# var-nan/SGUFP_Solver

Measured on AMD Instinct MI355X. Metric: B&B-node relaxations/sec + achieved HBM GB/s, 1k-arc 256-scenario synthetic, higher is better.
Workload: dtype f64; 1 GPU; C4: 1000-arc layered network, 256 scenarios, 16F+64O pool, BFS frontier of 8192 open nodes per GPU; instance_seed=1, nodes_per_gpu=8192, total_layers=281, parallelism=frontier shards x1

## Files before the change

include/sgufp_hip.h:

```cpp
#ifndef SGUFP_HIP_H
#define SGUFP_HIP_H

#include <stdint.h>

#ifdef __cplusplus
extern "C" {
#endif

typedef struct sgufp_ctx sgufp_ctx;

#define SGUFP_OK 0
#define SGUFP_ERR_ARG (-1)
#define SGUFP_ERR_NETWORK (-2)
#define SGUFP_ERR_HIP (-3)
#define SGUFP_ERR_CAPACITY (-4)
#define SGUFP_ERR_STATE (-5)
#define SGUFP_ERR_KEY (-6)

#define SGUFP_SUCCESS 0
#define SGUFP_PRUNED_BY_FEASIBILITY_CUT 1
#define SGUFP_PRUNED_BY_OPTIMALITY_CUT 2
#define SGUFP_NEEDS_SUBPROBLEM 3
#define SGUFP_PRUNED_BY_BOUND 4
#define SGUFP_NODE_ERR_RECORD 16
// ... 41 lines not shown
int sgufp_batch_children(sgufp_ctx *ctx, int64_t *child_off, uint16_t *global_layer, double *lb, double *ub,
                         int64_t *states_off, int16_t *states, int64_t *sol_off, int16_t *sol);
int sgufp_batch_paths(sgufp_ctx *ctx, int64_t *path_off, int16_t *paths);
int sgufp_batch_stats(sgufp_ctx *ctx, int64_t *dd_nodes, int64_t *dd_arcs, int32_t *dd_layers, int32_t *sweeps);
int sgufp_batch_refine(sgufp_ctx *ctx, int n, const int32_t *node_idx, const uint8_t *is_feasibility,
                       const int32_t *cut_index, double optimal_lb);

int sgufp_dd_build(sgufp_ctx *ctx);
int sgufp_dd_apply(sgufp_ctx *ctx, int node, int is_feasibility, double rhs, int64_t nnz, const uint64_t *keys,
                   const double *vals, double optimal, double *value);
int sgufp_dd_solution(sgufp_ctx *ctx, int node, int16_t *path, int32_t *len);
int sgufp_dd_cutset(sgufp_ctx *ctx, int node, double ub, int64_t *n_children);

int sgufp_batch_debug(sgufp_ctx *ctx, int64_t *ticks, int32_t *redo);
int sgufp_relax_launches(const sgufp_ctx *ctx, int64_t *launches);
int sgufp_batch_phases(sgufp_ctx *ctx, int64_t *phase);
int sgufp_batch_narrow_split(sgufp_ctx *ctx, int64_t *split);
int sgufp_batch_refold_stats(sgufp_ctx *ctx, uint32_t *stats);

#define SGUFP_ROUTE_IN_ORDER 0
#define SGUFP_ROUTE_EXACT_PHASE 1
#define SGUFP_ROUTE_NX_PHASE 2
#define SGUFP_ROUTE_NX_FALLBACK 3
int sgufp_batch_routes(sgufp_ctx *ctx, int32_t *route);

int sgufp_subproblem(sgufp_ctx *ctx, int n, const int64_t *path_off, const int16_t *paths, int32_t *type,
                     double *rhs, double *rows, double *obj_mean);
int sgufp_subproblem_detail(sgufp_ctx *ctx, int32_t *status, double *objective, double *dual_objective);
int sgufp_subproblem_warm(sgufp_ctx *ctx, int n, const int64_t *path_off, const int16_t *paths, const int32_t *warm_src,
                          const int32_t *warm_dst, int32_t *type, double *rhs, double *rows, double *obj_mean);
// ... 87 lines not shown
```

sgufp_solver_amd/csrc/capi.cpp:

```cpp
#include <cstdio>

#include "ctx.hpp"
#include <algorithm>
#include <cstdlib>


namespace {

int64_t node_bound(const Network &net, int64_t *tail = nullptr) {
    const int L = net.L;
    auto set_size = [&](int sid) { return sid >= 0 ? (int)net.sets[sid].size() : 1; };
    int start = std::max(0, L - 5);
    std::vector<int64_t> h(kMaxStates + 2, 0);
    int c0 = set_size(net.layer_universe[start]);
    h[c0] = (L > 5) ? kRelaxedMaxWidth - 1 : 1;
    int64_t total = (int64_t)(kRelaxedMaxWidth - 1) * (start + 1);
    int64_t tail_nodes = 0;
    for (int l = start; l < L; l++) {
        if (net.layer_update[l] >= 0) {
            int64_t w = 0;
            for (auto x : h) w += x;
            std::fill(h.begin(), h.end(), 0);
            h[set_size(net.layer_update[l])] = w;
        }
// ... 88 lines not shown
    if (const char *e = getenv("SGUFP_NX_MIN")) nx_min = std::max(1, atoi(e));
    if (const char *e = getenv("SGUFP_NX_SKIP")) nx_skip = std::max(0, atoi(e));
    if (const char *e = getenv("SGUFP_REDO_SWEEP")) sc.redo_sweep = atoi(e) != 0;
    if (const char *e = getenv("SGUFP_RELAX_CHUNK")) { split_q = std::max(0, atoi(e)); split_forced = true; }
    if (const char *e = getenv("SGUFP_RELAX_STREAMS")) split_parts = std::max(1, std::min(kRelaxMaxParts, atoi(e)));
    int64_t acap = std::max<int64_t>(1, (int64_t)std::max(0, L - 4) * (kRelaxedMaxWidth - 1) * maxU);
    if (ncap > (int64_t)kParentMask || acap > (int64_t)0x7FFFFFFF) { err = "DD capacity beyond 22-bit indices"; return false; }
    sc.Ncap = (int)ncap;
    sc.Acap = (int)acap;
    sc.us = ustride;
    if (net.n_slots >= 32767) { err = "more than 32766 coefficient slots (int16 root-solution slots)"; return false; }
    if (relax_lds_bytes(sc.Tcap, sc.Lcap, cb, sc.us) > 160 * 1024) { err = "too many layers for the LDS layer table"; return false; }
    sc.tmir_cap = cb > 1 ? (int)(sc.Ncap + sc.Acap) : 0;
    sc.tail_cap = (int)tail;
    sc.cb_max = cb;
    const size_t B = (size_t)max_batch;
    if (!alloc(sc.ntopo, B * sc.Ncap, "scratch") || !alloc(sc.nflag, B * sc.Ncap, "scratch") ||
        !alloc(sc.nmask, B * sc.Ncap, "scratch") || !alloc(sc.outcnt, B * sc.Ncap, "scratch") ||
        !alloc(sc.s2, B * sc.Ncap, "scratch") || !alloc(sc.tw, B * sc.Ncap, "scratch") ||
        !alloc(sc.atopo, B * sc.Acap, "scratch") || !alloc(sc.aflag, B * sc.Acap, "scratch") ||
        !alloc(sc.lay, B * sc.Tcap * 5, "scratch") || !alloc(sc.rslot, B * sc.Lcap, "scratch") ||
        !alloc(sc.meta, B * 8, "scratch") || !alloc(sc.ubv, B, "scratch") ||
        !alloc(sc.sm1, B * sc.Tcap, "scratch") || !alloc(sc.xm1, B * sc.Tcap, "scratch") ||
        !alloc(sc.v1, B * sc.Tcap, "scratch"))
        return false;
    if (cb > 1 && (!alloc(sc.s2b, B * sc.tail_cap * cb, "scratch") || !alloc(sc.sm, B * sc.Tcap * cb, "scratch") ||
                   !alloc(sc.xm, B * sc.Tcap * cb, "scratch") || !alloc(sc.tmir, B * (size_t)sc.tmir_cap, "scratch")))
        return false;
    if (cb > 1 && split_q > 0) {
        if (!alloc(sc.resume, B * kResumeWords, "scratch") || !alloc(sc.rgs, B * (size_t)(sc.Tcap + 1), "scratch")) return false;
        split_min = cus * relax_occupancy(sc.Tcap, sc.Lcap, cb, sc.us) * 3 / 2;
    }
    if (const char *e = getenv("SGUFP_REFOLD_STATS"))
        if (atoi(e) != 0 && cb > 1 && !alloc(sc.rstat, B * kRefoldStats, "scratch")) return false;
    if (!alloc(out.status, B, "out") || !alloc(out.exact, B, "out") || !alloc(out.lb, B, "out") ||
        !alloc(out.ub, B, "out") || !alloc(out.nchild, B, "out") || !alloc(out.sol_need, B, "out") ||
        !alloc(out.dd_nodes, B, "out") || !alloc(out.dd_arcs, B, "out") || !alloc(out.dd_layers, B, "out") ||
        !alloc(out.sweeps, B, "out") || !alloc(out.path, B * sc.Lcap, "out") || !alloc(out.path_len, B, "out") ||
        !alloc(out.ticks, B, "out") || !alloc(out.redo, B, "out") || !alloc(out.phase, B * kPhaseSlots, "out"))
        return false;
    if (!alloc(d_gl, B, "batch") || !alloc(d_sollen, B, "batch") || !alloc(d_lb, B, "batch") ||
        !alloc(d_ub, B, "batch") || !alloc(d_mask, B, "batch") || !alloc(d_valid, B, "batch") ||
        !alloc(d_soloff, B, "batch") || !alloc(d_coff, B + 1, "batch") || !alloc(d_soff, B + 1, "batch") ||
        !alloc(d_rslots, B, "batch") || !alloc(d_rcuts, B, "batch") || !alloc(d_rfeas, B, "batch"))
        return false;
    sol_cap = B * (size_t)std::max(1, L);
    if (!alloc(d_sol, sol_cap, "batch")) return false;
// ... 232 lines not shown
        if (!alloc(d_G, B * (size_t)ocap, "nx gaps") || !alloc(d_MS, B * (size_t)ocap, "nx maxState")) return false;
        nx_cap = ocap;
    }
    ex.nx = 1;
    ex.pkind = d_pkind;
    ex.P = d_P;
    ex.G = d_G;
    ex.MS = d_MS;
    ex.nxh = d_nxh;
    ex.pstop = d_pstop;
    ex.nxlist = d_nxlist;
    ex.nx_ms = 0;
    return true;
}

bool sgufp_ctx::split_prepare() {
    if (split_ready) return true;
    if (!hip_ok(hipEventCreateWithFlags(&split.fork, hipEventDisableTiming), "event")) return false;
    for (int k = 0; k + 1 < split_parts; k++)
        if (!hip_ok(hipStreamCreateWithFlags(&split.extra[k], hipStreamNonBlocking), "stream") ||
            !hip_ok(hipEventCreateWithFlags(&split.join[k], hipEventDisableTiming), "event"))
            return false;
    split_ready = true;
    return true;
}

bool sgufp_ctx::relax_current(double optimal_lb) {
    dd_built = false;
    if (!push_orders() || !exact_prepare()) return false;
    relax_lb = optimal_lb;
    BatchIn in = cur;
    if (!relax_order(in)) return false;
    const Pool p = pool();
    hipStream_t st = stream;
    const bool do_split = sc.resume && split_q > 0 && (split_forced || in.n >= split_min);
    if (do_split && !split_prepare()) return false;
    split.q = do_split ? split_q : 0;
    split.parts = split_parts;
    relax_launches = 0;
    split.launches = &relax_launches;
    if (timing) hipEventRecord(ev[0], st);
    if (!hip_ok(launch_relax(nd, sc, in, p, out, optimal_lb, cb, ex, cus, st, &split), "k_relax")) return false;
    if (timing) hipEventRecord(ev[1], st);
    return emit_current(in, p);
}

bool sgufp_ctx::emit_current(const BatchIn &in, const Pool &p) {
    hipStream_t st = stream;
    if (in.n > 0 && !hip_ok(launch_scan(out.nchild, out.sol_need, in.n, d_coff, d_soff, st), "k_scan2")) return false;
    uint64_t tot[2] = {0, 0};
    if (in.n > 0) {
        if (!download(&tot[0], d_coff + in.n, 1) || !download(&tot[1], d_soff + in.n, 1)) return false;
    }
    if (!sync()) return false;
    const char *es = std::getenv("SGUFP_EXACT_STATS");
    const bool estats = es && es[0] == '1';
    if (estats && ex.enabled) {
// ... 901 lines not shown
        const auto &v = is_feasibility[k] ? ctx->f_rows : ctx->o_rows;
        if (node_idx[k] < 0 || node_idx[k] >= ctx->n || cut_index[k] < 0 || cut_index[k] >= (int)v.size())
            return SGUFP_ERR_ARG;
        rows[k] = v[cut_index[k]];
    }
    if (!ctx->upload(ctx->d_rslots, node_idx, n) || !ctx->upload(ctx->d_rcuts, rows.data(), n) ||
        !ctx->upload(ctx->d_rfeas, is_feasibility, n))
        return SGUFP_ERR_HIP;
    if (!ctx->hip_ok(launch_refine(ctx->nd, ctx->sc, ctx->batch(), ctx->pool(), ctx->out, ctx->d_rslots, ctx->d_rcuts,
                                   ctx->d_rfeas, n, optimal_lb, ctx->ex, ctx->stream),
                     "k_refine"))
        return SGUFP_ERR_HIP;
    return ctx->sync() ? SGUFP_OK : SGUFP_ERR_HIP;
}

int sgufp_relax_launches(const sgufp_ctx *ctx, int64_t *launches) {
    if (!ctx || !launches) return SGUFP_ERR_ARG;
    if (!ctx->relaxed) return SGUFP_ERR_STATE;
    *launches = (int64_t)ctx->relax_launches;
    return SGUFP_OK;
}

int sgufp_batch_phases(sgufp_ctx *ctx, int64_t *phase) {
    if (!ctx || !ctx->relaxed || !phase) return ctx ? SGUFP_ERR_STATE : SGUFP_ERR_ARG;
    if (!relax_has_phases()) {
        std::fill(phase, phase + (size_t)ctx->n * 8, (int64_t)0);
        return SGUFP_OK;
    }
    std::vector<uint64_t> t((size_t)ctx->n * kPhaseSlots);
    if (!ctx->download(t.data(), ctx->out.phase, t.size()) || !ctx->sync()) return SGUFP_ERR_HIP;
// ... 206 lines not shown
```

sgufp_solver_amd/csrc/ctx.hpp:

```cpp
#pragma once

#include "sgufp_hip.h"

#include <hip/hip_runtime.h>

#include <algorithm>
#include <cstdlib>
#include <cstring>
#include <memory>
#include <string>
#include <unordered_map>
#include <vector>

#define SGUFP_HOST_ONLY 1
#include "dd_device.hpp"
#include "network.hpp"
#include "sub_device.hpp"
#include "rdd_device.hpp"
#include "select_device.hpp"

namespace sgufp {
struct Transport;
size_t relax_lds_bytes(int Tcap, int Lcap, int cb, int us);
size_t sub_lds_bytes(int n, int m, int nct_cap, int nz, int nw, int kbytes = 8, bool warm = false);
hipError_t launch_subproblem(const SubNet &N, const SubIO &io, hipStream_t st);
hipError_t launch_warm_pick(const SubIO &io, const WarmRing &wr, int ptr, hipStream_t st);
hipError_t launch_flow_summary(int P, int S, int m, const int32_t *reward, int16_t *x, const uint8_t *ok,
                               double *flow_reward, double *mean_flow, hipStream_t st);
hipError_t launch_relax(const NetDev &, const Scratch &, const BatchIn &, const Pool &, const BatchOut &, double, int,
                        const ExactIO &, int, hipStream_t, const RelaxSplit *);
int relax_occupancy(int Tcap, int Lcap, int cb, int us);
hipError_t launch_exact_cols(const double *rows, const double *rhs, const int32_t *o_order, int no, int first,
                             int stride, int n_slots, int ostride, double *coefO, int reverse, hipStream_t st);
hipError_t launch_scan(const uint32_t *, const uint32_t *, int, uint64_t *, uint64_t *, hipStream_t);
hipError_t launch_emit(const NetDev &, const Scratch &, const BatchIn &, const Pool &, const BatchOut &,
                       const ChildOut &, hipStream_t);
hipError_t launch_refine(const NetDev &, const Scratch &, const BatchIn &, const Pool &, const BatchOut &,
                         const int32_t *, const int32_t *, const uint8_t *, int, double, const ExactIO &, hipStream_t);
hipError_t launch_gather_paths(const BatchOut &, int Lcap, const int32_t *idx, const int64_t *off, int n,
                               int16_t *dst, hipStream_t);
hipError_t launch_push_children(const ChildOut &, const BatchOut &, const int32_t *parents, const int64_t *dst_child,
                                const int64_t *dst_sol, int n, const FrontierDev &, hipStream_t);
hipError_t launch_dd_build(const NetDev &, const Scratch &, const BatchIn &, const BatchOut &, int stride, hipStream_t);
hipError_t launch_dd_apply(const NetDev &, const Scratch &, const BatchIn &, const BatchOut &, int slot, const double *rows,
                           int stride, double rhs, int is_feas, double optimal, double *value, hipStream_t);
// ... 206 lines not shown
    unsigned long long leaf_cum[5] = {0, 0, 0, 0, 0};
    int32_t *d_open_cnt = nullptr, *d_open_list = nullptr;
    double *d_G = nullptr;
    unsigned long long *d_MS = nullptr;
    int nx_cap = 0;
    bool nx_prepare(int no);
    bool exact_prepare();

    int split_q = 32, split_parts = 2, split_min = 0;
    bool split_forced = false;
    RelaxSplit split{};
    bool split_ready = false;
    bool split_prepare();
    unsigned long long relax_launches = 0;

    bool timing = false;
    hipEvent_t ev[4] = {};
    float ms_relax = 0, ms_emit = 0;

    ~sgufp_ctx();
    void destroy_all() {
        if (device >= 0) (void)hipSetDevice(device);
        for (auto &b : allocs) (void)hipFree(b.p);
        for (auto &e : ev)
            if (e) (void)hipEventDestroy(e);
        if (split.fork) (void)hipEventDestroy(split.fork);
        for (auto &e : split.join)
            if (e) (void)hipEventDestroy(e);
        for (auto &s : split.extra)
            if (s) (void)hipStreamDestroy(s);
// ... 88 lines not shown
```

sgufp_solver_amd/csrc/dd_device.hpp:

```cpp
#pragma once

#include <cstdint>

#include <hip/hip_runtime_api.h>

#if defined(__HIP_DEVICE_COMPILE__) && !defined(SGUFP_HOST_ONLY)
#define SGUFP_GBL __attribute__((address_space(1)))
#else
#define SGUFP_GBL
#endif

namespace sgufp {

constexpr int kWave = 64;
constexpr int kMaxU = 32;
constexpr int kLdsWidth = 512;
constexpr int kBoundBlocks = 1024;

enum NodeStatus : int32_t {
    kSuccess = 0,
    kPrunedFeasibility = 1,
    kPrunedOptimality = 2,
    kNeedsSubproblem = 3,
    kPrunedBound = 4,
// ... 65 lines not shown

constexpr int kRelaxWhole = 0, kRelaxHead = 1, kRelaxChunk = 2;
constexpr int32_t kRelaxPending = 8;
struct RelaxPart {
    int first;
    int q;
};
constexpr int kRelaxMaxParts = 4;
struct RelaxSplit {
    int q, parts;
    hipStream_t extra[kRelaxMaxParts - 1];
    hipEvent_t fork, join[kRelaxMaxParts - 1];
    unsigned long long *launches;
};

struct BatchIn {
    int n;
    const uint16_t SGUFP_GBL *gl;
    const double SGUFP_GBL *lb;
    const double SGUFP_GBL *ub;
    const uint32_t SGUFP_GBL *mask;
    const uint8_t SGUFP_GBL *valid;
    const int64_t SGUFP_GBL *sol_off;
    const uint16_t SGUFP_GBL *sol_len;
    const int16_t SGUFP_GBL *sol;
    int bound_prune;
    const int32_t SGUFP_GBL *perm;
};

struct FrontierDev {
// ... 125 lines not shown
```

sgufp_solver_amd/csrc/dd_kernels.hip:

```cpp
#include <hip/hip_runtime.h>

#include <algorithm>
#include <climits>
#include <cstdint>
#include <type_traits>

#include "dd_device.hpp"
#include "wave.hpp"

namespace sgufp {

#define DMIN (-__DBL_MAX__)
#define DMAX (__DBL_MAX__)

constexpr uint32_t kCollapseWidth = 120;


struct VP {
    double v;
    int p;
};
__device__ __forceinline__ VP vp_pick(VP a, VP b) {
    const bool take_b = (a.p == INT_MIN) | ((b.p != INT_MIN) & ((b.v > a.v) | (!(a.v > b.v) & (b.p > a.p))));
    VP r;
// ... 1556 lines not shown
__device__ __forceinline__ void store_meta_layers(const DD &d, const Scratch &sc, int slot, int last_cut, int status,
                                         int cut_layer, double ub) {
    GBL int32_t *meta = sc.meta + (size_t)slot * 8;
    if (lane() == 0) {
        meta[0] = d.g; meta[1] = d.len; meta[2] = d.T; meta[3] = d.exact; meta[4] = d.aligned;
        meta[5] = last_cut; meta[6] = status; meta[7] = cut_layer;
        sc.ubv[slot] = ub;
    }
    GBL uint32_t *lay = sc.lay + (size_t)slot * sc.Tcap * 5;
    for (int k = lane(); k < d.T; k += kWave) {
        lay[k] = (d.noff[k]); lay[sc.Tcap + k] = (d.nn[k]); lay[2 * sc.Tcap + k] = (d.nalive[k]);
        lay[3 * sc.Tcap + k] = (d.aoff[k]); lay[4 * sc.Tcap + k] = (d.acnt[k]);
    }
}

__device__ __forceinline__ int dd_solution_path(const NetDev &net, DD &d, const GBL double *row, GBL int16_t *out_path,
                                const GBL int16_t *rsol) {
    const int last = d.T - 1;
    const uint32_t lo = uni(d.noff[last]), ln = uni(d.nn[last]);
    VP best{0.0, INT_MIN};
    for (uint32_t base = 0; base < ln; base += kWave) {
        uint32_t i = base + lane();
        if (i < ln && (d.nflag[lo + i] & kAlive)) best = vp_pick(best, VP{d.tw[lo + i], prio_old((int)i)});
    }
    best = wave_vp(best);
    uint32_t node = 0;
    int k = 0;
    if (best.p != INT_MIN && best.v > DMIN) {
        node = lo + (uint32_t)(-best.p - 2);
        k = last;
// ... 597 lines not shown
    bv.tring = (LDS uint16_t *)(smem + cv.o_tring);
    bv.coef = (LDS double *)(smem + cv.o_bcoef);
    bv.w1 = smem + cv.o_w1;
    bv.ids = (LDS int32_t *)(smem + cv.o_ids);
    bv.wm = (LDS uint64_t *)(smem + cv.o_wm);
    bv.fm = bv.wm + (sc.Tcap + 63) / 64;
    bv.wsel = nullptr;
    bv.s2b = sc.s2b + (size_t)slot * sc.tail_cap * CB;
    bv.sm = sc.sm + (size_t)slot * sc.Tcap * CB;
    bv.xm = sc.xm + (size_t)slot * sc.Tcap * CB;
    bv.rstat = sc.rstat ? sc.rstat + (size_t)slot * kRefoldStats : nullptr;
}

template <int CB, int MODE = kRelaxWhole>
__global__ void __launch_bounds__(kWave, 2) k_relax(NetDev net, Scratch sc, BatchIn in, Pool pool, BatchOut out,
                                                double incumbent, ExactIO ex, RelaxPart part) {
    static_assert(MODE == kRelaxWhole || CB > 1, "only the batched loop suspends");
    extern __shared__ __attribute__((aligned(16))) uint8_t smem_raw[];
    LDS uint8_t *smem = (LDS uint8_t *)smem_raw;
    constexpr bool chunk = MODE == kRelaxChunk;
    const int wg = part.first + (int)blockIdx.x;
    if (wg >= in.n) return;
    const int slot = in.perm ? in.perm[wg] : wg;
    if (MODE == kRelaxWhole && ex.redo && out.status[slot] != kNxFallback) return;
    if (chunk && out.status[slot] != kRelaxPending) return;
    if (!chunk && sc.rstat && lane() < kRefoldStats) sc.rstat[(size_t)slot * kRefoldStats + lane()] = 0;
#ifdef SGUFP_PHASES
    const uint64_t t_start = wall_clock64();
    uint64_t t_before = 0;
#endif
    DD d;
// ... 7 lines not shown
    d.len = uni((int)in.sol_len[slot]);
    const GBL int16_t *rsol = in.sol + in.sol_off[slot];
    d.aligned = (d.len == d.g) ? 1 : 0;
    int cut_layer = 0;
#ifdef SGUFP_PHASES
    LoopState st{kSuccess, in.ub[slot], -1, 0, 0, {0, 0, 0, 0, 0, 0, 0, 0}, t_start, {0, 0, 0}};
#else
    LoopState st{kSuccess, in.ub[slot], -1, 0, 0};
#endif
    double lb = DMIN;
    uint32_t nchild = 0, n_nodes = 0, n_arcs = 0, n_merged = 0;
    bool efast = false;
    int nx_k0 = -1;
    d.T = 1; d.exact = 1;
    LoopResume rs{0, false, false, pool.nf, false};

    if constexpr (chunk) {
        const GBL int32_t *rw = sc.resume + (size_t)slot * kResumeWords;
        load_meta_layers(d, sc, slot);
        rs.s = uni(rw[0]);
        rs.screened = (uni(rw[1]) & 1) != 0;
        rs.nx_tried = (uni(rw[1]) & 2) != 0;
        rs.limit = part.q > 0 ? rs.s + part.q : INT_MAX;
        st.applied = (uint32_t)uni(rw[2]);
        st.redo = (uint32_t)uni(rw[3]);
        st.last_cut = uni(sc.meta[(size_t)slot * 8 + 5]);
        st.ub = sc.ubv[slot];
        n_nodes = (uint32_t)uni(rw[8]); n_arcs = (uint32_t)uni(rw[9]); n_merged = (uint32_t)uni(rw[10]);
        LdsCarve cv = lds_carve(sc.Tcap, sc.Lcap, CB, sc.us);
        d.tmir = sc.tmir + (size_t)slot * sc.tmir_cap;
// ... 26 lines not shown
        goto done;
    }
    for (int t = lane(); t < d.len; t += kWave) {
        int dec = rsol[t];
        int s = -1;
        if (dec != -1) {
            s = net.n_slots;
            if (dec >= 0 && dec < net.m) {
                int j = net.arc_head[dec];
                for (int q = net.slot_off[t]; q < net.slot_off[t + 1]; q++)
                    if (net.slot_head[q] == j) { s = q; break; }
            }
        }
        d.rslot[t] = (int16_t)s;
    }
    if (!dd_build(net, d, sc, in.mask[slot], n_nodes, n_arcs, n_merged)) {
        st.status = kErrCapacity;
        goto done;
    }
    st.stamp(0);
    efast = ex.enabled && d.exact && pool.no > 0 && d.T <= kExactMaxT && (d.T - 1) * sc.us <= kExactMaxEntriesWide;
    if (CB > 1 && d.aligned) {
        LdsCarve cv = lds_carve(sc.Tcap, sc.Lcap, CB, sc.us);
        d.tmir = sc.tmir + (size_t)slot * sc.tmir_cap;
        d.gstart = (LDS uint16_t *)(smem + cv.o_gs);
        BatchView bv;
        relax_batch_view<CB>(bv, smem, cv, sc, slot);
        build_stream(d, n_merged, CB * pool.ustride);
        const bool nxtry = ex.enabled && ex.nx && !ex.redo && !d.exact && pool.no >= ex.nx_min;
        if (d.stream)
            cut_loop_batched<CB, MODE>(net, d, sc, bv, pool, incumbent, st, efast, nxtry ? &ex : nullptr, slot, &nx_k0, &rs);
        else cut_loop_single(net, d, pool, incumbent, 0, st, efast);
    } else {
        cut_loop_single(net, d, pool, incumbent, 0, st, efast);
    }
looped: __attribute__((unused));
    st.stamp(6);
    if (MODE != kRelaxWhole && rs.suspended) {
        if (lane() == 0) {
            GBL int32_t *rw = sc.resume + (size_t)slot * kResumeWords;
            rw[0] = rs.s; rw[1] = (rs.screened ? 1 : 0) | (rs.nx_tried ? 2 : 0);
            rw[2] = (int32_t)st.applied; rw[3] = (int32_t)st.redo;
            rw[4] = d.kg; rw[5] = (int32_t)d.Nn; rw[6] = (int32_t)d.Amir; rw[7] = d.ng;
// ... 515 lines not shown
            }
        }
    }
    if (status != kSuccess) ub = DMIN;
    if (lane() == 0) {
        out.status[slot] = status;
        out.lb[slot] = DMIN;
        out.ub[slot] = ub;
        out.nchild[slot] = nchild;
        out.sol_need[slot] = nchild * (uint32_t)(d.len + cut_layer);
        out.sweeps[slot] += (uint32_t)(pool.no - first);
    }
    store_meta_layers(d, sc, slot, last_cut, status, cut_layer, ub);
}

__global__ void __launch_bounds__(1024) k_scan2(const uint32_t *a, const uint32_t *b, int n, uint64_t *oa,
                                               uint64_t *ob) {
    __shared__ uint64_t sa[1024], sb[1024];
    const int t = threadIdx.x;
    const int per = (n + 1023) / 1024;
    const int lo = min(n, t * per), hi = min(n, lo + per);
    uint64_t xa = 0, xb = 0;
    for (int i = lo; i < hi; i++) { xa += a[i]; xb += b[i]; }
    sa[t] = xa; sb[t] = xb;
    __syncthreads();
    for (int d = 1; d < 1024; d <<= 1) {
        uint64_t ya = (t >= d) ? sa[t - d] : 0, yb = (t >= d) ? sb[t - d] : 0;
        __syncthreads();
        sa[t] += ya; sb[t] += yb;
        __syncthreads();
// ... 12 lines not shown
                        hipStream_t st);

int relax_occupancy(int Tcap, int Lcap, int cb, int us) {
    const size_t lds = relax_lds_bytes(Tcap, Lcap, cb, us);
    const auto k = cb == 4 ? k_relax<4> : cb == 8 ? k_relax<8> : cb == 16 ? k_relax<16> : k_relax<1>;
    int nb = 0;
    if (hipOccupancyMaxActiveBlocksPerMultiprocessor(&nb, k, kWave, lds) != hipSuccess) {
        (void)hipGetLastError();
        return 8;
    }
    return nb > 0 ? nb : 8;
}

template <int CB>
static hipError_t relax_split(const NetDev &net, const Scratch &sc, const BatchIn &in, const Pool &pool, const BatchOut &out,
                              double incumbent, const ExactIO &ex, const RelaxSplit &sp, size_t lds, hipStream_t st) {
    const int parts = std::max(1, std::min(sp.parts, std::min(in.n, kRelaxMaxParts)));
    const int nchunk = pool.no > 0 ? (pool.no + sp.q - 1) / sp.q : 0;
    hipError_t e;
    if (parts > 1 && (e = hipEventRecord(sp.fork, st)) != hipSuccess) return e;
    for (int p = 0; p < parts; p++) {
        const hipStream_t s = p == 0 ? st : sp.extra[p - 1];
        const int lo = (int)((int64_t)in.n * p / parts), hi = (int)((int64_t)in.n * (p + 1) / parts);
        if (p > 0 && (e = hipStreamWaitEvent(s, sp.fork, 0)) != hipSuccess) return e;
        BatchIn part = in;
        part.n = hi;
        hipLaunchKernelGGL((k_relax<CB, kRelaxHead>), dim3(hi - lo), dim3(kWave), lds, s, net, sc, part, pool, out, incumbent,
                           ex, RelaxPart{lo, 0});
        if (sp.launches) ++*sp.launches;
        for (int c = 0; c < nchunk; c++) {
            hipLaunchKernelGGL((k_relax<CB, kRelaxChunk>), dim3(hi - lo), dim3(kWave), lds, s, net, sc, part, pool, out,
                               incumbent, ex, RelaxPart{lo, c + 1 < nchunk ? sp.q : 0});
            if (sp.launches) ++*sp.launches;
        }
        if ((e = hipGetLastError()) != hipSuccess) return e;
        if (p > 0 && ((e = hipEventRecord(sp.join[p - 1], s)) != hipSuccess ||
                      (e = hipStreamWaitEvent(st, sp.join[p - 1], 0)) != hipSuccess))
            return e;
    }
    return hipSuccess;
}

hipError_t launch_relax(const NetDev &net, const Scratch &sc, const BatchIn &in, const Pool &pool,
                        const BatchOut &out, double incumbent, int cb, const ExactIO &ex, int cus, hipStream_t st,
                        const RelaxSplit *sp) {
    if (in.n <= 0) return hipSuccess;
    size_t lds = relax_lds_bytes(sc.Tcap, sc.Lcap, cb, sc.us);
    auto relax = [&](const ExactIO &io) {
        const auto k = cb == 4 ? k_relax<4> : cb == 8 ? k_relax<8> : cb == 16 ? k_relax<16> : k_relax<1>;
        hipLaunchKernelGGL(k, dim3(in.n), dim3(kWave), lds, st, net, sc, in, pool, out, incumbent, io, RelaxPart{0, 0});
        if (sp && sp->launches) ++*sp->launches;
        return hipGetLastError();
    };
    hipError_t e;
    if (sp && sp->q > 0 && sc.resume && (cb == 4 || cb == 8 || cb == 16))
        e = cb == 4 ? relax_split<4>(net, sc, in, pool, out, incumbent, ex, *sp, lds, st)
          : cb == 8 ? relax_split<8>(net, sc, in, pool, out, incumbent, ex, *sp, lds, st)
                    : relax_split<16>(net, sc, in, pool, out, incumbent, ex, *sp, lds, st);
    else
        e = relax(ex);
    if (e != hipSuccess || !ex.enabled || ex.no <= 0) return e;
    if ((e = launch_exact(net, sc, ex, incumbent, cus, st)) != hipSuccess) return e;
    hipLaunchKernelGGL(k_exact_fin, dim3(in.n), dim3(kWave), relax_lds_bytes(sc.Tcap, sc.Lcap, 1, sc.us), st, net, sc, in,
                       pool, out, ex, incumbent);
    if ((e = hipGetLastError()) != hipSuccess || !ex.nx || !ex.pkind) return e;
    hipLaunchKernelGGL(k_nx_fin, dim3(in.n), dim3(kWave), relax_lds_bytes(sc.Tcap, sc.Lcap, 1, sc.us), st, net, sc, in,
                       pool, out, ex, incumbent);
    if ((e = hipGetLastError()) != hipSuccess) return e;
    ExactIO rx = ex;
    rx.redo = 1;
    return relax(rx);
}

hipError_t launch_scan(const uint32_t *a, const uint32_t *b, int n, uint64_t *oa, uint64_t *ob, hipStream_t st) {
    hipLaunchKernelGGL(k_scan2, dim3(1), dim3(1024), 0, st, a, b, n, oa, ob);
    return hipGetLastError();
}

hipError_t launch_emit(const NetDev &net, const Scratch &sc, const BatchIn &in, const Pool &pool,
                       const BatchOut &out, const ChildOut &co, hipStream_t st) {
    if (in.n <= 0) return hipSuccess;
    size_t lds = relax_lds_bytes(sc.Tcap, sc.Lcap, 1, sc.us);
    hipLaunchKernelGGL(k_emit_children, dim3(in.n), dim3(kWave), lds, st, net, sc, in, pool, out, co);
    return hipGetLastError();
}

// ... 1 lines not shown
#ifdef SGUFP_PHASES
    return true;
#else
    return false;
#endif
}

hipError_t launch_dd_build(const NetDev &net, const Scratch &sc, const BatchIn &in, const BatchOut &out, int stride,
                           hipStream_t st) {
    if (in.n <= 0) return hipSuccess;
    Pool none{};
    none.stride = stride;
    none.ustride = 1;
    ExactIO ex{};
    hipLaunchKernelGGL(k_relax<1>, dim3(in.n), dim3(kWave), relax_lds_bytes(sc.Tcap, sc.Lcap, 1, sc.us), st, net, sc,
                       in, none, out, DMIN, ex, RelaxPart{0, 0});
    return hipGetLastError();
}

hipError_t launch_dd_apply(const NetDev &net, const Scratch &sc, const BatchIn &in, const BatchOut &out, int slot,
                           const double *rows, int stride, double rhs, int is_feas, double optimal, double *value,
                           hipStream_t st) {
    hipLaunchKernelGGL(k_dd_apply, dim3(1), dim3(kWave), relax_lds_bytes(sc.Tcap, sc.Lcap, 1, sc.us), st, net, sc, in,
                       out, slot, rows, stride, rhs, is_feas, optimal, value);
    return hipGetLastError();
}

hipError_t launch_dd_solution(const NetDev &net, const Scratch &sc, const BatchIn &in, const BatchOut &out, int slot,
                              const double *rows, int stride, hipStream_t st) {
    hipLaunchKernelGGL(k_dd_solution, dim3(1), dim3(kWave), relax_lds_bytes(sc.Tcap, sc.Lcap, 1, sc.us), st, net, sc,
                       in, out, slot, rows, stride);
// ... 22 lines not shown
```

sgufp_solver_amd/engine.py:

```python
from __future__ import annotations

import ctypes as C
import os
from typing import List, Optional, Sequence, Tuple

import numpy as np

from .pools import DOUBLE_MIN, NodeRecord, PoolCut, RelaxResult

HERE = os.path.dirname(os.path.abspath(__file__))
LIB_PATH = os.environ.get("SGUFP_LIB_PATH") or os.path.join(HERE, "lib", "libsgufp_hip.so")

SUCCESS, PRUNED_F, PRUNED_O, NEEDS_SUBPROBLEM, PRUNED_BOUND = 0, 1, 2, 3, 4
ROUTE_IN_ORDER, ROUTE_EXACT_PHASE, ROUTE_NX_PHASE, ROUTE_NX_FALLBACK = 0, 1, 2, 3
ERR_RECORD, ERR_CAPACITY, ERR_CUTSET = 16, 17, 18

EXPORTS = [
    "sgufp_create_from_file", "sgufp_create", "sgufp_destroy", "sgufp_get_network_info",
    "sgufp_processing_order", "sgufp_last_error", "sgufp_stream", "sgufp_cuts_append",
    "sgufp_cuts_clear", "sgufp_cuts_count", "sgufp_batch_upload", "sgufp_batch_relax",
    "sgufp_batch_sync", "sgufp_batch_results", "sgufp_batch_children_size", "sgufp_batch_children",
    "sgufp_batch_paths", "sgufp_batch_stats", "sgufp_batch_refine", "sgufp_set_timing",
    "sgufp_last_timing", "sgufp_probe_network", "sgufp_batch_debug",
    "sgufp_batch_phases", "sgufp_batch_narrow_split", "sgufp_batch_refold_stats", "sgufp_subproblem", "sgufp_subproblem_detail", "sgufp_slot_keys",
# ... 88 lines not shown
    lib.sgufp_batch_children.argtypes = [P, P, P, P, P, P, P, P, P]
    lib.sgufp_batch_paths.argtypes = [P, P, P]
    lib.sgufp_batch_stats.argtypes = [P, P, P, P, P]
    lib.sgufp_batch_refine.argtypes = [P, C.c_int, P, P, P, C.c_double]
    lib.sgufp_set_timing.argtypes = [P, C.c_int]
    lib.sgufp_last_timing.argtypes = [P, P, P]
    lib.sgufp_probe_network.argtypes = [C.c_char_p, P, P, C.c_int32, P, P]
    lib.sgufp_batch_debug.argtypes = [P, P, P]
    lib.sgufp_batch_phases.argtypes = [P, P]
    lib.sgufp_batch_narrow_split.argtypes = [P, P]
    if hasattr(lib, "sgufp_batch_refold_stats"):
        lib.sgufp_batch_refold_stats.argtypes = [P, P]
    lib.sgufp_batch_routes.argtypes = [P, P]
    if hasattr(lib, "sgufp_relax_launches"):
        lib.sgufp_relax_launches.argtypes = [P, P]
    lib.sgufp_subproblem.argtypes = [P, C.c_int, P, P, P, P, P, P]
    lib.sgufp_subproblem_detail.argtypes = [P, P, P, P]
    lib.sgufp_slot_keys.argtypes = [P, P]
    lib.sgufp_cuts_append_rows.argtypes = [P, C.c_int, C.c_int, P, P]
    lib.sgufp_frontier_clear.argtypes = [P]
    lib.sgufp_frontier_size.argtypes = [P, P, P]
    lib.sgufp_frontier_push.argtypes = [P, C.c_int, P, P, P, P, P, P, P]
    lib.sgufp_frontier_take_size.argtypes = [P, C.c_int, C.c_int, P, P]
    lib.sgufp_frontier_take.argtypes = [P, C.c_int, C.c_int, P, P, P, P, P, P, P]
    lib.sgufp_bnb_step.argtypes = [P, C.c_int, P, P]
    lib.sgufp_balance_plan.argtypes = [C.c_int, P, P, P, P, P]
    lib.sgufp_comm_allgather_i64.argtypes = [P, P, C.c_int, P]
    lib.sgufp_frontier_peek_size.argtypes = [P, C.c_int64, C.c_int, P, P]
    lib.sgufp_frontier_peek.argtypes = [P, C.c_int64, C.c_int, P, P, P, P, P, P, P]
    lib.sgufp_bnb_set_limits.argtypes = [P, C.c_int, C.c_double]
# ... 272 lines not shown
    def phases(self):
        t = np.zeros((self.n, 8), dtype=np.int64)
        self._check(self.lib.sgufp_batch_phases(self.ctx, _ptr(t)))
        return t

    def narrow_split(self):
        t = np.zeros((self.n, 3), dtype=np.int64)
        self._check(self.lib.sgufp_batch_narrow_split(self.ctx, _ptr(t)))
        return t

    def relax_launches(self) -> int:
        v = C.c_int64(0)
        self._check(self.lib.sgufp_relax_launches(self.ctx, C.byref(v)))
        return int(v.value)

    def refold_stats(self):
        t = np.zeros((self.n, 16), dtype=np.uint32)
        self._check(self.lib.sgufp_batch_refold_stats(self.ctx, _ptr(t)))
        return t

    def children_batch(self) -> BatchArrays:
        child_off, gl, lb, ub, soff, states, poff, sol = self.children_arrays()
        return batch_from_arrays(gl, lb, ub, soff, states[:soff[-1]], poff, sol[:poff[-1]])

    def paths(self):
        n = self.n
        off = np.zeros(n + 1, dtype=np.int64)
        self._check(self.lib.sgufp_batch_paths(self.ctx, _ptr(off), None))
        buf = np.zeros(max(int(off[-1]), 1), dtype=np.int16)
        self._check(self.lib.sgufp_batch_paths(self.ctx, _ptr(off), _ptr(buf)))
# ... 310 lines not shown
```

Before: 390,900 relaxations/s.

## Share DD builds across batch nodes with identical layer/mask via device templates

Before relaxation, frontier nodes are hashed on (global layer, mask). Each key that appears at least twice gets a pre-built decision-diagram template, built once per kernel launch. Matching nodes then copy the template's topology, flags and layer tables with vectorized copies instead of running dd_build and build_stream themselves. This adds three small kernels, a memset, template memory and copy traffic, and it only pays off when many nodes share keys.

Result: faster. 415,100 relaxations/s, median of 6 (+6.2%).

```diff
diff --git a/include/sgufp_hip.h b/include/sgufp_hip.h
--- a/include/sgufp_hip.h
+++ b/include/sgufp_hip.h
@@ -79,6 +79,7 @@
 
 int sgufp_batch_debug(sgufp_ctx *ctx, int64_t *ticks, int32_t *redo);
 int sgufp_relax_launches(const sgufp_ctx *ctx, int64_t *launches);
+int sgufp_relax_templates(sgufp_ctx *ctx, int64_t *built, int64_t *instantiated);
 int sgufp_batch_phases(sgufp_ctx *ctx, int64_t *phase);
 int sgufp_batch_narrow_split(sgufp_ctx *ctx, int64_t *split);
 int sgufp_batch_refold_stats(sgufp_ctx *ctx, uint32_t *stats);
diff --git a/sgufp_solver_amd/csrc/capi.cpp b/sgufp_solver_amd/csrc/capi.cpp
--- a/sgufp_solver_amd/csrc/capi.cpp
+++ b/sgufp_solver_amd/csrc/capi.cpp
@@ -126,7 +126,7 @@
     sc.tmir_cap = cb > 1 ? (int)(sc.Ncap + sc.Acap) : 0;
     sc.tail_cap = (int)tail;
     sc.cb_max = cb;
-    const size_t B = (size_t)max_batch;
+    const size_t B = (size_t)max_batch, held0 = held;
     if (!alloc(sc.ntopo, B * sc.Ncap, "scratch") || !alloc(sc.nflag, B * sc.Ncap, "scratch") ||
         !alloc(sc.nmask, B * sc.Ncap, "scratch") || !alloc(sc.outcnt, B * sc.Ncap, "scratch") ||
         !alloc(sc.s2, B * sc.Ncap, "scratch") || !alloc(sc.tw, B * sc.Ncap, "scratch") ||
@@ -143,6 +143,8 @@
         if (!alloc(sc.resume, B * kResumeWords, "scratch") || !alloc(sc.rgs, B * (size_t)(sc.Tcap + 1), "scratch")) return false;
         split_min = cus * relax_occupancy(sc.Tcap, sc.Lcap, cb, sc.us) * 3 / 2;
     }
+    if (const char *e = getenv("SGUFP_RELAX_TEMPLATES")) tpl_mode = atoi(e) != 0 ? 1 : 0;
+    if (cb > 1 && (tpl_mode == 1 || (tpl_mode < 0 && sc.resume)) && !tpl_init(held - held0)) return false;
     if (const char *e = getenv("SGUFP_REFOLD_STATS"))
         if (atoi(e) != 0 && cb > 1 && !alloc(sc.rstat, B * kRefoldStats, "scratch")) return false;
     if (!alloc(out.status, B, "out") || !alloc(out.exact, B, "out") || !alloc(out.lb, B, "out") ||
@@ -405,6 +407,34 @@
     return true;
 }
 
+bool sgufp_ctx::tpl_init(size_t scratch_bytes) {
+    Scratch &tp = tpl.tp;
+    tp = sc;
+    const size_t slot_bytes = (size_t)sc.Ncap * 13 + (size_t)sc.Acap * 5 + (size_t)sc.tmir_cap * 2 +
+                              (size_t)sc.Tcap * 22 + kResumeWords * 4 + 8 * 4 + 8 + 8;
+    int64_t K = std::max<int64_t>(16, (int64_t)(scratch_bytes / 20 / slot_bytes));
+    if (const char *e = getenv("SGUFP_RELAX_TEMPLATE_SLOTS")) K = std::max(1, atoi(e));
+    K = std::min<int64_t>(K, max_batch);
+    const size_t k = (size_t)K;
+    tp.rstat = nullptr;
+    if (!alloc(tp.ntopo, k * sc.Ncap, "templates") || !alloc(tp.nflag, k * sc.Ncap + 4, "templates") ||
+        !alloc(tp.nmask, k * sc.Ncap, "templates") || !alloc(tp.outcnt, k * sc.Ncap, "templates") ||
+        !alloc(tp.atopo, k * sc.Acap, "templates") || !alloc(tp.aflag, k * sc.Acap + 4, "templates") ||
+        !alloc(tp.tmir, k * (size_t)sc.tmir_cap + 2, "templates") || !alloc(tp.lay, k * sc.Tcap * 5, "templates") ||
+        !alloc(tp.rgs, k * (size_t)(sc.Tcap + 1), "templates") || !alloc(tp.resume, k * kResumeWords, "templates") ||
+        !alloc(tp.meta, k * 8, "templates") || !alloc(tp.ubv, k, "templates") || !alloc(tpl.tkey, k, "templates") ||
+        !alloc(tpl.rec, (size_t)max_batch, "templates"))
+        return false;
+    tpl_table_cap = 64;
+    while (tpl_table_cap < 2 * max_batch) tpl_table_cap *= 2;
+    unsigned long long *tab = nullptr;
+    if (!alloc(tab, 2 + (size_t)tpl_table_cap * 2, "templates")) return false;
+    tpl.ctr = tab;
+    tpl.keys = tab + 2;
+    tpl.K = (int)K;
+    return true;
+}
+
 bool sgufp_ctx::split_prepare() {
     if (split_ready) return true;
     if (!hip_ok(hipEventCreateWithFlags(&split.fork, hipEventDisableTiming), "event")) return false;
@@ -430,8 +460,16 @@
     split.parts = split_parts;
     relax_launches = 0;
     split.launches = &relax_launches;
+    tpl_used = tpl.K > 0 && (tpl_mode == 1 || (tpl_mode < 0 && do_split && in.n >= split_min));
+    if (tpl_used) {
+        tpl.table = 64;
+        while (tpl.table < 2 * in.n) tpl.table *= 2;
+        tpl.count = (uint32_t *)(tpl.keys + tpl.table);
+        tpl.tid = (int32_t *)(tpl.count + tpl.table);
+    }
     if (timing) hipEventRecord(ev[0], st);
-    if (!hip_ok(launch_relax(nd, sc, in, p, out, optimal_lb, cb, ex, cus, st, &split), "k_relax")) return false;
+    if (!hip_ok(launch_relax(nd, sc, in, p, out, optimal_lb, cb, ex, cus, st, &split, tpl_used ? &tpl : nullptr), "k_relax"))
+        return false;
     if (timing) hipEventRecord(ev[1], st);
     return emit_current(in, p);
 }
@@ -1363,6 +1401,17 @@
     return ctx->sync() ? SGUFP_OK : SGUFP_ERR_HIP;
 }
 
+int sgufp_relax_templates(sgufp_ctx *ctx, int64_t *built, int64_t *instantiated) {
+    if (!ctx || !built || !instantiated) return SGUFP_ERR_ARG;
+    *built = *instantiated = 0;
+    if (!ctx->tpl_used) return SGUFP_OK;
+    unsigned long long c[2] = {0, 0};
+    if (!ctx->download(c, ctx->tpl.ctr, 2) || !ctx->sync()) return SGUFP_ERR_HIP;
+    *built = (int64_t)std::min<unsigned long long>(c[0], (unsigned long long)ctx->tpl.K);
+    *instantiated = (int64_t)c[1];
+    return SGUFP_OK;
+}
+
 int sgufp_relax_launches(const sgufp_ctx *ctx, int64_t *launches) {
     if (!ctx || !launches) return SGUFP_ERR_ARG;
     if (!ctx->relaxed) return SGUFP_ERR_STATE;
diff --git a/sgufp_solver_amd/csrc/ctx.hpp b/sgufp_solver_amd/csrc/ctx.hpp
--- a/sgufp_solver_amd/csrc/ctx.hpp
+++ b/sgufp_solver_amd/csrc/ctx.hpp
@@ -28,7 +28,7 @@
 hipError_t launch_flow_summary(int P, int S, int m, const int32_t *reward, int16_t *x, const uint8_t *ok,
                                double *flow_reward, double *mean_flow, hipStream_t st);
 hipError_t launch_relax(const NetDev &, const Scratch &, const BatchIn &, const Pool &, const BatchOut &, double, int,
-                        const ExactIO &, int, hipStream_t, const RelaxSplit *);
+                        const ExactIO &, int, hipStream_t, const RelaxSplit *, const Templates *);
 int relax_occupancy(int Tcap, int Lcap, int cb, int us);
 hipError_t launch_exact_cols(const double *rows, const double *rhs, const int32_t *o_order, int no, int first,
                              int stride, int n_slots, int ostride, double *coefO, int reverse, hipStream_t st);
@@ -265,6 +265,12 @@
     bool split_prepare();
     unsigned long long relax_launches = 0;
 
+    Templates tpl{};
+    int tpl_mode = -1;
+    int tpl_table_cap = 0;
+    bool tpl_used = false;
+    bool tpl_init(size_t scratch_bytes);
+
     bool timing = false;
     hipEvent_t ev[4] = {};
     float ms_relax = 0, ms_emit = 0;
diff --git a/sgufp_solver_amd/csrc/dd_device.hpp b/sgufp_solver_amd/csrc/dd_device.hpp
--- a/sgufp_solver_amd/csrc/dd_device.hpp
+++ b/sgufp_solver_amd/csrc/dd_device.hpp
@@ -103,6 +103,19 @@
     unsigned long long *launches;
 };
 
+struct Templates {
+    int K;
+    int table;
+    unsigned long long SGUFP_GBL *ctr;
+    unsigned long long SGUFP_GBL *keys;
+    uint32_t SGUFP_GBL *count;
+    int32_t SGUFP_GBL *tid;
+    int32_t SGUFP_GBL *rec;
+    unsigned long long SGUFP_GBL *tkey;
+    Scratch tp;
+};
+constexpr int kTplOk = 11;
+
 struct BatchIn {
     int n;
     const uint16_t SGUFP_GBL *gl;
diff --git a/sgufp_solver_amd/csrc/dd_kernels.hip b/sgufp_solver_amd/csrc/dd_kernels.hip
--- a/sgufp_solver_amd/csrc/dd_kernels.hip
+++ b/sgufp_solver_amd/csrc/dd_kernels.hip
@@ -1594,6 +1594,86 @@
     }
 }
 
+typedef uint32_t u32x4a __attribute__((ext_vector_type(4), aligned(4)));
+typedef double f64x2a __attribute__((ext_vector_type(2), aligned(8)));
+constexpr int kCopyUnroll = 4;
+
+__device__ __forceinline__ void copy_words(GBL uint32_t *__restrict__ dst, const GBL uint32_t *__restrict__ src, uint32_t n) {
+    const uint32_t n4 = n >> 2;
+    GBL u32x4a *d4 = (GBL u32x4a *)dst;
+    const GBL u32x4a *s4 = (const GBL u32x4a *)src;
+    for (uint32_t base = 0; base < n4; base += kCopyUnroll * kWave) {
+        u32x4a v[kCopyUnroll];
+#pragma unroll
+        for (int u = 0; u < kCopyUnroll; u++) {
+            const uint32_t i = base + (uint32_t)u * kWave + (uint32_t)lane();
+            if (i < n4) v[u] = s4[i];
+        }
+#pragma unroll
+        for (int u = 0; u < kCopyUnroll; u++) {
+            const uint32_t i = base + (uint32_t)u * kWave + (uint32_t)lane();
+            if (i < n4) d4[i] = v[u];
+        }
+    }
+    for (uint32_t i = (n4 << 2) + (uint32_t)lane(); i < n; i += kWave) dst[i] = src[i];
+}
+__device__ __forceinline__ void copy_bytes(GBL uint8_t *__restrict__ dst, const GBL uint8_t *__restrict__ src, uint32_t n) {
+    const uint32_t head = min(n, (uint32_t)(-(uintptr_t)dst & 3u));
+    if ((uint32_t)lane() < head) dst[lane()] = src[lane()];
+    const uint32_t nw = (n - head) >> 2;
+    GBL uint32_t *dw = (GBL uint32_t *)(dst + head);
+    const uint32_t sh = (uint32_t)((uintptr_t)(src + head) & 3u);
+    if (sh == 0) {
+        copy_words(dw, (const GBL uint32_t *)(src + head), nw);
+    } else {
+        const GBL uint32_t *sw = (const GBL uint32_t *)(src + head - sh);
+#pragma unroll kCopyUnroll
+        for (uint32_t i = lane(); i < nw; i += kWave) dw[i] = __builtin_amdgcn_alignbyte(sw[i + 1], sw[i], sh);
+    }
+    const uint32_t done = head + (nw << 2);
+    if ((uint32_t)lane() < n - done) dst[done + lane()] = src[done + lane()];
+}
+__device__ __forceinline__ void fill_f64(GBL double *dst, uint32_t n, double x) {
+    const uint32_t n2 = n >> 1;
+    GBL f64x2a *d2 = (GBL f64x2a *)dst;
+    const f64x2a v = {x, x};
+    for (uint32_t i = lane(); i < n2; i += kWave) d2[i] = v;
+    if ((n & 1u) && lane() == 0) dst[n - 1] = x;
+}
+
+__device__ __forceinline__ bool dd_instantiate(DD &d, const Templates &tpl, int t, uint32_t &n_nodes, uint32_t &n_arcs,
+                                               uint32_t &n_merged) {
+    const Scratch &tp = tpl.tp;
+    const GBL int32_t *tw = tp.resume + (size_t)t * kResumeWords;
+    if (!uni(tw[kTplOk])) return false;
+    d.T = uni(tw[0]); d.exact = uni(tw[1]);
+    d.kg = uni(tw[4]); d.Nn = (uint32_t)uni(tw[5]); d.Amir = (uint32_t)uni(tw[6]); d.ng = uni(tw[7]);
+    n_nodes = (uint32_t)uni(tw[8]); n_arcs = (uint32_t)uni(tw[9]); n_merged = (uint32_t)uni(tw[10]);
+    const GBL uint32_t *lay = tp.lay + (size_t)t * tp.Tcap * 5;
+    for (int k = lane(); k < d.T; k += kWave) {
+        d.noff[k] = lay[k]; d.nn[k] = lay[tp.Tcap + k]; d.nalive[k] = lay[2 * tp.Tcap + k];
+        d.aoff[k] = lay[3 * tp.Tcap + k]; d.acnt[k] = lay[4 * tp.Tcap + k];
+    }
+    const GBL uint16_t *gs = tp.rgs + (size_t)t * (tp.Tcap + 1);
+    for (int k = lane(); k <= d.ng; k += kWave) d.gstart[k] = gs[k];
+    const size_t N = (size_t)t * tp.Ncap, A = (size_t)t * tp.Acap;
+    const uint32_t nodes = n_nodes - 1;
+    copy_words(d.ntopo, tp.ntopo + N, nodes);
+    copy_words(d.nmask, tp.nmask + N, nodes);
+    copy_words(d.outcnt, tp.outcnt + N, nodes);
+    copy_words(d.atopo, tp.atopo + A, n_merged);
+    copy_bytes((GBL uint8_t *)d.tmir, (const GBL uint8_t *)(tp.tmir + (size_t)t * tp.tmir_cap), 2u * (d.Nn + d.Amir));
+    copy_bytes(d.nflag, tp.nflag + N, nodes);
+    copy_bytes(d.aflag, tp.aflag + A, n_merged);
+    fill_f64(d.s2, nodes, DMIN);
+    wave_lds_sync();
+    const uint32_t lo = uni(d.noff[d.T - 1]), ln = uni(d.nn[d.T - 1]);
+    for (uint32_t i = lane(); i < ln; i += kWave) d.tw[lo + i] = DMAX;
+    d.stream = 1;
+    wave_mem_sync();
+    return true;
+}
+
 __device__ __forceinline__ int dd_solution_path(const NetDev &net, DD &d, const GBL double *row, GBL int16_t *out_path,
                                 const GBL int16_t *rsol) {
     const int last = d.T - 1;
@@ -2221,7 +2301,7 @@
 
 template <int CB, int MODE = kRelaxWhole>
 __global__ void __launch_bounds__(kWave, 2) k_relax(NetDev net, Scratch sc, BatchIn in, Pool pool, BatchOut out,
-                                                double incumbent, ExactIO ex, RelaxPart part) {
+                                                double incumbent, ExactIO ex, RelaxPart part, Templates tpl) {
     static_assert(MODE == kRelaxWhole || CB > 1, "only the batched loop suspends");
     extern __shared__ __attribute__((aligned(16))) uint8_t smem_raw[];
     LDS uint8_t *smem = (LDS uint8_t *)smem_raw;
@@ -2259,6 +2339,7 @@
     int nx_k0 = -1;
     d.T = 1; d.exact = 1;
     LoopResume rs{0, false, false, pool.nf, false};
+    bool copied = false;
 
     if constexpr (chunk) {
         const GBL int32_t *rw = sc.resume + (size_t)slot * kResumeWords;
@@ -2315,7 +2396,17 @@
         }
         d.rslot[t] = (int16_t)s;
     }
-    if (!dd_build(net, d, sc, in.mask[slot], n_nodes, n_arcs, n_merged)) {
+    if (CB > 1 && !chunk && tpl.K > 0 && d.aligned) {
+        const int e = uni(tpl.rec[slot]);
+        const int t = e >= 0 ? uni(tpl.tid[e]) - 1 : -1;
+        if (t >= 0) {
+            d.tmir = sc.tmir + (size_t)slot * sc.tmir_cap;
+            d.gstart = (LDS uint16_t *)(smem + lds_carve(sc.Tcap, sc.Lcap, CB, sc.us).o_gs);
+            copied = dd_instantiate(d, tpl, t, n_nodes, n_arcs, n_merged);
+            if (copied && lane() == 0) atomicAdd(&tpl.ctr[1], 1ull);
+        }
+    }
+    if (!copied && !dd_build(net, d, sc, in.mask[slot], n_nodes, n_arcs, n_merged)) {
         st.status = kErrCapacity;
         goto done;
     }
@@ -2327,7 +2418,7 @@
         d.gstart = (LDS uint16_t *)(smem + cv.o_gs);
         BatchView bv;
         relax_batch_view<CB>(bv, smem, cv, sc, slot);
-        build_stream(d, n_merged, CB * pool.ustride);
+        if (!copied) build_stream(d, n_merged, CB * pool.ustride);
         const bool nxtry = ex.enabled && ex.nx && !ex.redo && !d.exact && pool.no >= ex.nx_min;
         if (d.stream)
             cut_loop_batched<CB, MODE>(net, d, sc, bv, pool, incumbent, st, efast, nxtry ? &ex : nullptr, slot, &nx_k0, &rs);
@@ -2873,6 +2964,69 @@
     store_meta_layers(d, sc, slot, last_cut, status, cut_layer, ub);
 }
 
+__global__ void __launch_bounds__(256) k_tpl_key(NetDev net, BatchIn in, Templates tpl, int Lcap, double incumbent) {
+    const int i = (int)(blockIdx.x * blockDim.x + threadIdx.x);
+    if (i >= in.n) return;
+    const int g = in.gl[i], len = in.sol_len[i];
+    int e = -1;
+    if (in.valid[i] && len == g && g <= net.L && len <= Lcap && !(in.bound_prune && in.ub[i] <= incumbent)) {
+        const unsigned long long key = (((unsigned long long)g << 32) | in.mask[i]) + 1ull;
+        const uint32_t m = (uint32_t)tpl.table - 1u;
+        uint32_t h = (uint32_t)((key * 0x9E3779B97F4A7C15ull) >> 32) & m;
+        for (;;) {
+            const unsigned long long old = atomicCAS(&tpl.keys[h], 0ull, key);
+            if (old == 0ull || old == key) break;
+            h = (h + 1u) & m;
+        }
+        atomicAdd(&tpl.count[h], 1u);
+        e = (int)h;
+    }
+    tpl.rec[i] = e;
+}
+__global__ void __launch_bounds__(256) k_tpl_assign(Templates tpl) {
+    const int e = (int)(blockIdx.x * blockDim.x + threadIdx.x);
+    if (e >= tpl.table || tpl.count[e] < 2u) return;
+    const unsigned long long id = atomicAdd(&tpl.ctr[0], 1ull);
+    if (id >= (unsigned long long)tpl.K) return;
+    tpl.tid[e] = (int32_t)id + 1;
+    tpl.tkey[id] = tpl.keys[e] - 1ull;
+}
+__global__ void __launch_bounds__(kWave) k_tpl_build(NetDev net, Templates tpl, int cb, int ustride) {
+    extern __shared__ __attribute__((aligned(16))) uint8_t smem_raw[];
+    LDS uint8_t *smem = (LDS uint8_t *)smem_raw;
+    const int t = (int)blockIdx.x;
+    const unsigned long long made = tpl.ctr[0];
+    if (t >= tpl.K || (unsigned long long)t >= made) return;
+    const Scratch &tp = tpl.tp;
+    const unsigned long long key = tpl.tkey[t];
+    DD d;
+    dd_bind(d, smem, tp, t, cb);
+    d.g = uni((int)(key >> 32));
+    d.len = d.g;
+    d.aligned = 1;
+    d.T = 1; d.exact = 1;
+    d.tmir = tp.tmir + (size_t)t * tp.tmir_cap;
+    d.gstart = (LDS uint16_t *)(smem + lds_carve(tp.Tcap, tp.Lcap, cb, tp.us).o_gs);
+    uint32_t n_nodes = 0, n_arcs = 0, n_merged = 0;
+    GBL int32_t *tw = tp.resume + (size_t)t * kResumeWords;
+    bool ok = dd_build(net, d, tp, (uint32_t)key, n_nodes, n_arcs, n_merged);
+    if (ok) {
+        build_stream(d, n_merged, cb * ustride);
+        ok = d.stream != 0;
+    }
+    if (ok) {
+        GBL uint16_t *gs = tp.rgs + (size_t)t * (tp.Tcap + 1);
+        for (int k = lane(); k <= d.ng; k += kWave) gs[k] = d.gstart[k];
+        store_meta_layers(d, tp, t, -1, kSuccess, 0, DMIN);
+        if (lane() == 0) {
+            tw[0] = d.T; tw[1] = d.exact; tw[2] = 0; tw[3] = 0;
+            tw[4] = d.kg; tw[5] = (int32_t)d.Nn; tw[6] = (int32_t)d.Amir; tw[7] = d.ng;
+            tw[8] = (int32_t)n_nodes; tw[9] = (int32_t)n_arcs; tw[10] = (int32_t)n_merged;
+        }
+    }
+    if (lane() == 0) tw[kTplOk] = ok ? 1 : 0;
+}
+
 __global__ void __launch_bounds__(1024) k_scan2(const uint32_t *a, const uint32_t *b, int n, uint64_t *oa,
                                                uint64_t *ob) {
     __shared__ uint64_t sa[1024], sb[1024];
@@ -2915,7 +3069,8 @@
 
 template <int CB>
 static hipError_t relax_split(const NetDev &net, const Scratch &sc, const BatchIn &in, const Pool &pool, const BatchOut &out,
-                              double incumbent, const ExactIO &ex, const RelaxSplit &sp, size_t lds, hipStream_t st) {
+                              double incumbent, const ExactIO &ex, const RelaxSplit &sp, size_t lds, hipStream_t st,
+                              const Templates &tpl) {
     const int parts = std::max(1, std::min(sp.parts, std::min(in.n, kRelaxMaxParts)));
     const int nchunk = pool.no > 0 ? (pool.no + sp.q - 1) / sp.q : 0;
     hipError_t e;
@@ -2927,11 +3082,11 @@
         BatchIn part = in;
         part.n = hi;
         hipLaunchKernelGGL((k_relax<CB, kRelaxHead>), dim3(hi - lo), dim3(kWave), lds, s, net, sc, part, pool, out, incumbent,
-                           ex, RelaxPart{lo, 0});
+                           ex, RelaxPart{lo, 0}, tpl);
         if (sp.launches) ++*sp.launches;
         for (int c = 0; c < nchunk; c++) {
             hipLaunchKernelGGL((k_relax<CB, kRelaxChunk>), dim3(hi - lo), dim3(kWave), lds, s, net, sc, part, pool, out,
-                               incumbent, ex, RelaxPart{lo, c + 1 < nchunk ? sp.q : 0});
+                               incumbent, ex, RelaxPart{lo, c + 1 < nchunk ? sp.q : 0}, Templates{});
             if (sp.launches) ++*sp.launches;
         }
         if ((e = hipGetLastError()) != hipSuccess) return e;
@@ -2944,22 +3099,33 @@
 
 hipError_t launch_relax(const NetDev &net, const Scratch &sc, const BatchIn &in, const Pool &pool,
                         const BatchOut &out, double incumbent, int cb, const ExactIO &ex, int cus, hipStream_t st,
-                        const RelaxSplit *sp) {
+                        const RelaxSplit *sp, const Templates *tp) {
     if (in.n <= 0) return hipSuccess;
     size_t lds = relax_lds_bytes(sc.Tcap, sc.Lcap, cb, sc.us);
-    auto relax = [&](const ExactIO &io) {
+    auto relax = [&](const ExactIO &io, const Templates &tpl) {
         const auto k = cb == 4 ? k_relax<4> : cb == 8 ? k_relax<8> : cb == 16 ? k_relax<16> : k_relax<1>;
-        hipLaunchKernelGGL(k, dim3(in.n), dim3(kWave), lds, st, net, sc, in, pool, out, incumbent, io, RelaxPart{0, 0});
+        hipLaunchKernelGGL(k, dim3(in.n), dim3(kWave), lds, st, net, sc, in, pool, out, incumbent, io, RelaxPart{0, 0},
+                           tpl);
         if (sp && sp->launches) ++*sp->launches;
         return hipGetLastError();
     };
     hipError_t e;
+    Templates tpl{};
+    if (tp && tp->K > 0 && (cb == 4 || cb == 8 || cb == 16)) {
+        tpl = *tp;
+        const size_t zero = 2 * sizeof(unsigned long long) + (size_t)tpl.table * (sizeof(unsigned long long) + 2 * sizeof(uint32_t));
+        if ((e = hipMemsetAsync((void *)tpl.ctr, 0, zero, st)) != hipSuccess) return e;
+        hipLaunchKernelGGL(k_tpl_key, dim3((in.n + 255) / 256), dim3(256), 0, st, net, in, tpl, sc.Lcap, incumbent);
+        hipLaunchKernelGGL(k_tpl_assign, dim3((tpl.table + 255) / 256), dim3(256), 0, st, tpl);
+        hipLaunchKernelGGL(k_tpl_build, dim3(tpl.K), dim3(kWave), lds, st, net, tpl, cb, pool.ustride);
+        if ((e = hipGetLastError()) != hipSuccess) return e;
+    }
     if (sp && sp->q > 0 && sc.resume && (cb == 4 || cb == 8 || cb == 16))
-        e = cb == 4 ? relax_split<4>(net, sc, in, pool, out, incumbent, ex, *sp, lds, st)
-          : cb == 8 ? relax_split<8>(net, sc, in, pool, out, incumbent, ex, *sp, lds, st)
-                    : relax_split<16>(net, sc, in, pool, out, incumbent, ex, *sp, lds, st);
+        e = cb == 4 ? relax_split<4>(net, sc, in, pool, out, incumbent, ex, *sp, lds, st, tpl)
+          : cb == 8 ? relax_split<8>(net, sc, in, pool, out, incumbent, ex, *sp, lds, st, tpl)
+                    : relax_split<16>(net, sc, in, pool, out, incumbent, ex, *sp, lds, st, tpl);
     else
-        e = relax(ex);
+        e = relax(ex, tpl);
     if (e != hipSuccess || !ex.enabled || ex.no <= 0) return e;
     if ((e = launch_exact(net, sc, ex, incumbent, cus, st)) != hipSuccess) return e;
     hipLaunchKernelGGL(k_exact_fin, dim3(in.n), dim3(kWave), relax_lds_bytes(sc.Tcap, sc.Lcap, 1, sc.us), st, net, sc, in,
@@ -2970,7 +3136,7 @@
     if ((e = hipGetLastError()) != hipSuccess) return e;
     ExactIO rx = ex;
     rx.redo = 1;
-    return relax(rx);
+    return relax(rx, Templates{});
 }
 
 hipError_t launch_scan(const uint32_t *a, const uint32_t *b, int n, uint64_t *oa, uint64_t *ob, hipStream_t st) {
@@ -3002,7 +3168,7 @@
     none.ustride = 1;
     ExactIO ex{};
     hipLaunchKernelGGL(k_relax<1>, dim3(in.n), dim3(kWave), relax_lds_bytes(sc.Tcap, sc.Lcap, 1, sc.us), st, net, sc,
-                       in, none, out, DMIN, ex, RelaxPart{0, 0});
+                       in, none, out, DMIN, ex, RelaxPart{0, 0}, Templates{});
     return hipGetLastError();
 }
 
diff --git a/sgufp_solver_amd/engine.py b/sgufp_solver_amd/engine.py
--- a/sgufp_solver_amd/engine.py
+++ b/sgufp_solver_amd/engine.py
@@ -126,6 +126,8 @@
     lib.sgufp_batch_routes.argtypes = [P, P]
     if hasattr(lib, "sgufp_relax_launches"):
         lib.sgufp_relax_launches.argtypes = [P, P]
+    if hasattr(lib, "sgufp_relax_templates"):
+        lib.sgufp_relax_templates.argtypes = [P, P, P]
     lib.sgufp_subproblem.argtypes = [P, C.c_int, P, P, P, P, P, P]
     lib.sgufp_subproblem_detail.argtypes = [P, P, P, P]
     lib.sgufp_slot_keys.argtypes = [P, P]
@@ -428,6 +430,11 @@
         self._check(self.lib.sgufp_relax_launches(self.ctx, C.byref(v)))
         return int(v.value)
 
+    def relax_templates(self):
+        b, i = C.c_int64(0), C.c_int64(0)
+        self._check(self.lib.sgufp_relax_templates(self.ctx, C.byref(b), C.byref(i)))
+        return int(b.value), int(i.value)
+
     def refold_stats(self):
         t = np.zeros((self.n, 16), dtype=np.uint32)
         self._check(self.lib.sgufp_batch_refold_stats(self.ctx, _ptr(t)))
```
